# facebookresearch/ReAgent

Measured on NVIDIA H100. Metric: minibatch_td_updates_per_sec_b4096, higher is better.
Workload: dtype f32

## Files before the change

### include/reagent_b200.h

```cpp
#ifndef REAGENT_B200_H_
#define REAGENT_B200_H_

#include <stdint.h>

#ifdef __cplusplus
extern "C" {
#endif

#define RB200_VERSION 1
#define RB200_MAX_LAYERS 8

#define RB200_OK 0
#define RB200_E_INVALID (-1)
#define RB200_E_CUDA (-2)
#define RB200_E_SMEM (-3)

#define RB200_ACT_LINEAR 0
#define RB200_ACT_RELU 1
#define RB200_ACT_TANH 2
#define RB200_ACT_LEAKY_RELU 3
#define RB200_ACT_SIGMOID 4
#define RB200_ACT_SOFTPLUS 5

#define RB200_LOSS_MSE 0
// ... 270 lines not shown
#define RB200_ALGO_TD3 1
typedef struct rb200_ac_args {
  int32_t batch;
  int32_t algo;
  const float* state;
  const float* action;
  const float* next_state;
  const float* reward;
  const float* not_terminal;
  const float* noise_next;
  const float* noise_cur;
  float gamma;
  const float* alpha;
  const float* log_alpha;
  float target_entropy;
  int32_t backprop_through_log_prob;
  float noise_variance, noise_clip;
  float* loss_partials;
  float* loss;
  uint32_t* tile_counter;
  float* alpha_grad;
  float* td_target;
  float* next_action_out;
  float* log_prob_out;
  float* q1_value;
  float* q2_value;
  const rb200_mlp_t* value_target;
  const rb200_mlp_t* value_net;
  float* min_q_out;
  int32_t crr_mode;
  float crr_threshold;
  float crr_beta;
  float crr_clamp;
  int32_t logged_action_uniform_prior;
  const float* sample_weight;
  float* td_error_out;
} rb200_ac_args_t;
#define RB200_CRR_NONE 0
#define RB200_CRR_INDICATOR 1
#define RB200_CRR_EXPONENT 2

int rb200_ac_critic_step(const rb200_mlp_t* actor, const rb200_mlp_t* q1, const rb200_mlp_t* q2,
                         const rb200_mlp_t* q1_target, const rb200_mlp_t* q2_target,
                         const rb200_ac_args_t* args, const rb200_net_ws_t* ws_q1,
                         const rb200_net_ws_t* ws_q2, void* stream);
int rb200_ac_actor_step(const rb200_mlp_t* actor, const rb200_mlp_t* q1, const rb200_mlp_t* q2,
                        const rb200_ac_args_t* args, const rb200_net_ws_t* ws_actor,
                        const rb200_net_ws_t* ws_q1, const rb200_net_ws_t* ws_q2, void* stream);
int rb200_ac_value_step(const rb200_mlp_t* value, const rb200_ac_args_t* args,
                        const rb200_net_ws_t* ws_value, void* stream);

int rb200_wgrad_splits(int batch);
int rb200_wgrad_splits_for(const rb200_mlp_t* net, int32_t batch);
int rb200_mlp_wgrad(const rb200_mlp_t* net, const float* net_input, int32_t batch,
                    const rb200_net_ws_t* ws, float* gpart, int32_t splits, void* stream);
int rb200_grad_reduce(const float* gpart, int32_t splits, int64_t n, float* g, void* stream);

typedef struct rb200_adam_args {
  float* params;
  const float* grad;
  int32_t splits;
  int64_t n;
  float* exp_avg;
  float* exp_avg_sq;
  int64_t* step;
  uint32_t* block_counter;
  double lr, beta1, beta2, eps, weight_decay;
  float grad_scale;
  float* target;
  float tau;
  float one_minus_tau;
  float* exp_out;
  const rb200_mlp_t* tc_net;
  void* tc_pack_ws;
  int64_t tc_pack_ws_bytes;
  int32_t tc_do_backward;
  int32_t dp_world, dp_rank;
  float* const* dp_recv;
  uint32_t* const* dp_flags;
  int64_t dp_stride;
  int32_t dp_max_blocks;
  int32_t decoupled_weight_decay;
  int32_t amsgrad;
  float* max_exp_avg_sq;
} rb200_adam_args_t;
int rb200_adam_blocks(int64_t n);
int rb200_adam_soft_update(const rb200_adam_args_t* a, void* stream);
int rb200_soft_update(float* target, const float* source, int64_t n, float tau,
                      float one_minus_tau, void* stream);


#define RB200_SAMPLE_PRIORITIZED 0
#define RB200_SAMPLE_UNIFORM 1
#define RB200_SAMPLE_GIVEN 2
#define RB200_VALID_BLOCK 256
#define RB200_MAX_GATHER_SPECS 12

typedef struct rb200_gather_spec {
  const void* src;
  void* dst;
  int32_t row_bytes;
  int32_t which;
} rb200_gather_spec_t;

typedef struct rb200_sample_args {
  int32_t batch, capacity, update_horizon, mode;
// ... 127 lines not shown
```

### reagent_b200/_lib.py

```python
import ctypes as C
import os

MAX_LAYERS = 8

ACT = {"linear": 0, "relu": 1, "tanh": 2, "leaky_relu": 3, "sigmoid": 4, "softplus": 5}
E_SMEM = -3
LOSS_MSE, LOSS_HUBER = 0, 1
DISCOUNT_CONST, DISCOUNT_POW = 0, 1

_f32p = C.POINTER(C.c_float)
_vp = C.c_void_p


class MlpT(C.Structure):
    _fields_ = [
        ("n_layers", C.c_int32),
        ("dims", C.c_int32 * (MAX_LAYERS + 1)),
        ("act", C.c_int32 * MAX_LAYERS),
        ("params", _vp),
        ("w_off", C.c_int64 * MAX_LAYERS),
        ("b_off", C.c_int64 * MAX_LAYERS),
        ("n_params", C.c_int64),
    ]

# ... 240 lines not shown
    lib.rb200_device_info.argtypes = [C.POINTER(C.c_int), C.POINTER(C.c_int)]
    lib.rb200_num_row_tiles.argtypes = [C.c_int, C.c_int, C.c_int]
    lib.rb200_dqn_td_step.argtypes = [C.POINTER(MlpT), C.POINTER(MlpT), C.POINTER(DqnArgsT),
                                      C.POINTER(NetWsT), _vp]
    lib.rb200_dueling_scratch_floats.argtypes = [C.c_int32, C.c_int32]
    lib.rb200_dueling_scratch_floats.restype = C.c_int64
    lib.rb200_dueling_fold.argtypes = [_vp, _vp, _vp, _vp, C.c_int32, C.c_int32, C.c_int32, _vp, _vp,
                                       _vp, _vp]
    lib.rb200_dueling_unfold.argtypes = [_vp, C.c_int64, C.c_int32, C.c_int32, C.c_int32, C.c_int32,
                                         C.c_int64, C.c_int64, C.c_int64, C.c_int64, C.c_int64,
                                         C.c_int64, _vp, _vp]
    lib.rb200_dqn_tc_workspace_bytes.argtypes = [C.POINTER(MlpT), C.c_int32, C.c_int32]
    lib.rb200_dqn_tc_workspace_bytes.restype = C.c_int64
    lib.rb200_dqn_tc_pack.argtypes = [C.POINTER(MlpT), C.POINTER(MlpT), C.c_int32, C.c_int32, _vp,
                                      C.c_int64, _vp]
    lib.rb200_dqn_td_step_tc.argtypes = [C.POINTER(MlpT), C.POINTER(MlpT), C.POINTER(DqnArgsT),
                                         C.POINTER(NetWsT), _vp, C.c_int64, C.c_int32, _vp]
    lib.rb200_mlp_forward.argtypes = [C.POINTER(MlpT), _vp, C.c_int32, _vp, C.c_int32, C.c_int32,
                                      _vp, C.POINTER(NetWsT), _vp]
    lib.rb200_mlp_forward_tiled.argtypes = [C.POINTER(MlpT), C.POINTER(MlpT), _vp, C.c_int32, _vp,
                                            C.c_int32, C.c_int32, C.c_int32, _vp, _vp, _vp]
    lib.rb200_linear_forward.argtypes = [_vp, _vp, C.c_int32, C.c_int32, C.c_int32, _vp,
                                         C.c_int32, _vp, _vp]
    lib.rb200_linear_backward_dx.argtypes = [_vp, C.c_int32, C.c_int32, _vp, _vp, C.c_int32,
                                             C.c_int32, _vp, _vp]
    lib.rb200_linear_backward_dx_tc_scratch_bytes.argtypes = [C.c_int32, C.c_int32, C.c_int32]
    lib.rb200_linear_backward_dx_tc_scratch_bytes.restype = C.c_int64
    lib.rb200_linear_backward_dx_tc.argtypes = [_vp, C.c_int32, C.c_int32, _vp, _vp, C.c_int32,
                                                C.c_int32, _vp, _vp, C.c_int64, _vp]
    lib.rb200_mlp_backward.argtypes = [C.POINTER(MlpT), _vp, C.c_int32, C.POINTER(NetWsT), _vp]
    lib.rb200_qrdqn_head.argtypes = [C.POINTER(QrdqnArgsT), _vp]
    lib.rb200_preprocess.argtypes = [_vp, _vp, C.c_int32, C.c_int64, C.c_int32, C.c_int32, _vp,
                                     _vp, _vp, _vp]
    lib.rb200_replay_sample.argtypes = [C.POINTER(SampleArgsT), _vp]
    lib.rb200_valid_index_build.argtypes = [_vp, C.c_int64, _vp, _vp, _vp]
    lib.rb200_mt19937_uniform_host.argtypes = [_vp, C.POINTER(C.c_int32), _vp, _vp, _vp, C.c_int64]
    lib.rb200_mt19937_uniform_host.restype = None
    lib.rb200_sumtree_set_host.argtypes = [_vp, C.c_int32, _vp, _vp, C.c_int64, _vp]
    lib.rb200_sumtree_sample_host.argtypes = [_vp, C.c_int32, C.c_double]
    lib.rb200_sumtree_sample_host.restype = C.c_int64
    lib.rb200_sumtree_sample_many_host.argtypes = [_vp, C.c_int32, _vp, _vp, C.c_int64, _vp]
    lib.rb200_sumtree_sample_many_host.restype = None
    lib.rb200_replay_add_batch_host.argtypes = [_vp, C.c_int64, C.c_int64, C.c_int32, _vp, _vp, _vp]
    lib.rb200_replay_add_batch_host.restype = None
    lib.rb200_ac_critic_step.argtypes = [C.POINTER(MlpT), C.POINTER(MlpT), C.POINTER(MlpT),
                                         C.POINTER(MlpT), C.POINTER(MlpT), C.POINTER(AcArgsT),
                                         C.POINTER(NetWsT), C.POINTER(NetWsT), _vp]
    lib.rb200_ac_actor_step.argtypes = [C.POINTER(MlpT), C.POINTER(MlpT), C.POINTER(MlpT),
                                        C.POINTER(AcArgsT), C.POINTER(NetWsT), C.POINTER(NetWsT),
                                        C.POINTER(NetWsT), _vp]
    lib.rb200_ac_value_step.argtypes = [C.POINTER(MlpT), C.POINTER(AcArgsT), C.POINTER(NetWsT), _vp]
    lib.rb200_wgrad_splits.argtypes = [C.c_int]
    lib.rb200_wgrad_splits_for.argtypes = [C.POINTER(MlpT), C.c_int32]
    lib.rb200_mlp_wgrad.argtypes = [C.POINTER(MlpT), _vp, C.c_int32, C.POINTER(NetWsT), _vp,
                                    C.c_int32, _vp]
    lib.rb200_grad_reduce.argtypes = [_vp, C.c_int32, C.c_int64, _vp, _vp]
    lib.rb200_adam_soft_update.argtypes = [C.POINTER(AdamArgsT), _vp]
    lib.rb200_soft_update.argtypes = [_vp, _vp, C.c_int64, C.c_float, C.c_float, _vp]
    lib.rb200_cpe_heads.argtypes = [C.POINTER(CpeArgsT), _vp]
    lib.rb200_bcq_filter.argtypes = [_vp, C.c_int32, C.c_int32, C.c_float, _vp, _vp, _vp, _vp, _vp]
    lib.rb200_pdqn_head.argtypes = [C.POINTER(PdqnArgsT), _vp]
    lib.rb200_c51_head.argtypes = [C.POINTER(C51ArgsT), _vp]
    lib.rb200_bc_xent_head.argtypes = [C.POINTER(BcXentArgsT), _vp]
    lib.rb200_crr_critic_head.argtypes = [C.POINTER(CrrCriticArgsT), _vp]
    lib.rb200_crr_actor_head.argtypes = [C.POINTER(CrrActorArgsT), _vp]
    lib.rb200_replay_add_device.argtypes = [C.POINTER(AddArgsT), _vp]
    lib.rb200_sumtree_set_device.argtypes = [_vp, C.c_int32, _vp, _vp, C.c_int32, _vp, _vp, _vp]
    lib.rb200_per_draw_indices.argtypes = [C.POINTER(PerDrawArgsT), _vp]
    lib.rb200_per_weights.argtypes = [_vp, C.c_int32, _vp, C.c_int32, _vp, C.c_double, C.c_double,
                                      _vp, _vp, _vp]
    lib.rb200_per_priority_update.argtypes = [_vp, C.c_int32, _vp, _vp, _vp, C.c_int32, C.c_double,
                                              C.c_double, _vp, _vp, _vp, _vp]
    lib.rb200_per_priority_update_rows.argtypes = [_vp, C.c_int32, _vp, _vp, C.c_int32, C.c_double,
                                                   C.c_double, C.c_double, _vp, _vp, _vp, _vp]
    lib.rb200_adam_blocks.argtypes = [C.c_int64]
    lib.rb200_dp_alloc.argtypes = [C.c_int64, C.POINTER(_vp)]
    lib.rb200_dp_free.argtypes = [_vp]
    lib.rb200_dp_ipc_handle.argtypes = [_vp, _vp]
    lib.rb200_dp_ipc_open.argtypes = [_vp, C.POINTER(_vp)]
    lib.rb200_dp_ipc_close.argtypes = [_vp]


def lib():
    global _LIB
    if _LIB is None:
        if not os.path.exists(LIB_PATH):
            raise Rb200Error(
                f"{LIB_PATH} not found: the CUDA extension is not built. "
                "Run reagent_b200/csrc/build.sh (there is no CPU fallback).")
        _LIB = C.CDLL(LIB_PATH)
        _declare(_LIB)
    return _LIB


def check(rc, what=""):
    if rc != 0:
        msg = lib().rb200_last_error().decode("utf-8", "replace")
        raise Rb200Error(f"{what} failed (rc={rc}): {msg}")


def ptr(t, device=None):
    if t is None:
        return None
    if not t.is_cuda:
        raise Rb200Error("reagent_b200: a CPU tensor reached a CUDA entry point (call "
                         "trainer.cuda() / batch.cuda() first; there is no CPU path)")
# ... 25 lines not shown
```

### reagent_b200/csrc/rb200_optim.cu

```cuda
#include <math.h>

#include <stdlib.h>

#include "rb200_dqn_tc_layout.cuh"

namespace rb200 {

constexpr int kWgTile = 64;
constexpr int kWgRows = 32;
constexpr int kWgLd = kWgTile + 8;

struct WgradLayer {
  const float* A;
  const float* dZ;
  int K, N;
  long long w_off, b_off;
  int tiles_n, tiles_k, tile_start;
};
struct WgradParams {
  int n_layers;
  WgradLayer L[kMaxLayers];
  int B, splits, rows_per_split;
  float* gpart;
  long long P;
// ... 273 lines not shown
    m = w1_small ? fmaf(w1, gm, m) : fmaf(w1m1, gm, g);
    v = __fadd_rn(__fmul_rn(v, b2), __fmul_rn(__fmul_rn(w2, g), g));
    float vd = v;
    if (kAmsgrad) {
      vd = fmax_nan(a.max_exp_avg_sq[i], v);
      a.max_exp_avg_sq[i] = vd;
    }
    const float denom = __fadd_rn(__fdiv_rn(__fsqrt_rn(vd), bc2_sqrt), eps);
    p = __fadd_rn(p, __fdiv_rn(__fmul_rn(-step_size, m), denom));
    a.params[i] = p;
    a.exp_avg[i] = m;
    a.exp_avg_sq[i] = v;
    if (a.exp_out) a.exp_out[i] = expf(p);
    float tn = 0.f;
    if (a.target) {
      const float tg = a.target[i];
      tn = __fadd_rn(__fmul_rn(a.tau, p), __fmul_rn(a.one_minus_tau, tg));
      a.target[i] = tn;
    }
    if (d.pv.pack) adam_pack_weight(d.pv, i, p, a.target != nullptr, tn);
  }
  __syncthreads();
  if (threadIdx.x == 0) {
    __threadfence();
    const unsigned done = atomicAdd(a.block_counter, 1u);
    if (done == gridDim.x - 1) {
      *a.step = t;
      *a.block_counter = 0u;
    }
  }
}

__global__ void soft_update_kernel(float* __restrict__ target, const float* __restrict__ src,
                                   long long n, float tau, float omt) {
  const long long stride = (long long)gridDim.x * blockDim.x;
  for (long long i = (long long)blockIdx.x * blockDim.x + threadIdx.x; i < n; i += stride)
    target[i] = __fadd_rn(__fmul_rn(tau, src[i]), __fmul_rn(omt, target[i]));
}

}

using namespace rb200;

extern "C" int rb200_wgrad_splits(int batch) {
  const char* e = getenv("RB200_WGRAD_ROWS");
  int rows = e ? atoi(e) : 256;
  if (rows < 32) rows = 32;
  int s = batch / rows;
  if (s < 1) s = 1;
  if (s > 64) s = 64;
  return s;
}

int rb200_wgrad_tc_launch(const rb200_mlp_t* net, const float* net_input, int32_t batch,
                          const rb200_net_ws_t* ws, float* gpart, int32_t splits, void* stream);

static bool wgrad_use_tc() {
  const char* d = getenv("RB200_DISABLE_WGMMA");
  const char* w = getenv("RB200_WGRAD_TC");
  return !(d && d[0] && d[0] != '0') && (w && w[0] == '1');
}

extern "C" int rb200_wgrad_splits_for(const rb200_mlp_t* net, int32_t batch) {
  if (!net || !wgrad_use_tc()) return rb200_wgrad_splits(batch);
  int jobs = 0;
  for (int l = 0; l < net->n_layers; ++l) jobs += ceil_div(net->dims[l + 1], 128) * ceil_div(net->dims[l], 256);
  int s = ceil_div(2 * kNumSMs, jobs < 1 ? 1 : jobs);
  const int smax = batch / 128 < 1 ? 1 : batch / 128;
  if (s > smax) s = smax;
  if (s > 64) s = 64;
  return s < 1 ? 1 : s;
}

extern "C" int rb200_mlp_wgrad(const rb200_mlp_t* net, const float* net_input, int32_t batch,
                               const rb200_net_ws_t* ws, float* gpart, int32_t splits,
                               void* stream) {
  if (!net || !ws || !gpart) { set_last_error("rb200_mlp_wgrad: null argument"); return RB200_E_INVALID; }
  if (int rc = validate_mlp(net, "net")) return rc;
  if (batch <= 0 || splits <= 0) { set_last_error("rb200_mlp_wgrad: bad batch/splits"); return RB200_E_INVALID; }
  if (wgrad_use_tc()) return rb200_wgrad_tc_launch(net, net_input, batch, ws, gpart, splits, stream);
  WgradParams p = {};
  p.n_layers = net->n_layers;
  p.B = batch;
  p.splits = splits;
  p.rows_per_split = ceil_div(ceil_div(batch, splits), kWgRows) * kWgRows;
  p.gpart = gpart;
  p.P = net->n_params;
  int tiles = 0;
  for (int l = 0; l < net->n_layers; ++l) {
    WgradLayer& L = p.L[l];
    L.A = (l == 0) ? (net_input ? net_input : ws->input) : ws->hidden[l - 1];
    L.dZ = ws->dz[l];
    if (!L.A || !L.dZ) { set_last_error("rb200_mlp_wgrad: missing activation / dz for layer %d", l); return RB200_E_INVALID; }
    L.K = net->dims[l];
    L.N = net->dims[l + 1];
    L.w_off = net->w_off[l];
    L.b_off = net->b_off[l];
    L.tiles_n = ceil_div(L.N, kWgTile);
    L.tiles_k = ceil_div(L.K, kWgTile);
    L.tile_start = tiles;
    tiles += L.tiles_n * L.tiles_k;
  }
  for (int l = net->n_layers; l < kMaxLayers; ++l) p.L[l].tile_start = 1 << 30;
  dim3 grid(tiles, splits);
  wgrad_kernel<<<grid, kThreads, 0, (cudaStream_t)stream>>>(p);
  return check_cuda(cudaGetLastError(), "wgrad_kernel launch");
}

extern "C" int rb200_grad_reduce(const float* gpart, int32_t splits, int64_t n, float* g,
                                 void* stream) {
  if (!gpart || !g || n <= 0 || splits <= 0) { set_last_error("rb200_grad_reduce: bad argument"); return RB200_E_INVALID; }
  int blocks = (int)((n + 255) / 256);
  if (blocks > kNumSMs * 8) blocks = kNumSMs * 8;
  grad_reduce_kernel<<<blocks, 256, 0, (cudaStream_t)stream>>>(gpart, splits, (long long)n, g);
  return check_cuda(cudaGetLastError(), "grad_reduce_kernel launch");
}

extern "C" int rb200_adam_soft_update(const rb200_adam_args_t* a, void* stream) {
  if (!a || !a->params || !a->grad || !a->exp_avg || !a->exp_avg_sq || !a->step || !a->block_counter) {
    set_last_error("rb200_adam_soft_update: null argument"); return RB200_E_INVALID;
  }
  if (a->n <= 0 || a->splits <= 0) { set_last_error("rb200_adam_soft_update: bad n/splits"); return RB200_E_INVALID; }
  if ((a->decoupled_weight_decay != 0 && a->decoupled_weight_decay != 1) ||
      (a->amsgrad != 0 && a->amsgrad != 1)) {
    set_last_error("rb200_adam_soft_update: decoupled_weight_decay and amsgrad must be 0 or 1"); return RB200_E_INVALID;
  }
  if (a->amsgrad && !a->max_exp_avg_sq) { set_last_error("rb200_adam_soft_update: amsgrad needs max_exp_avg_sq"); return RB200_E_INVALID; }
  AdamDev d;
  d.a = *a;
  d.a.tc_net = nullptr;
  d.pv.pack = nullptr;
  if (a->tc_net && a->tc_pack_ws) {
    const rb200_mlp_t* q = a->tc_net;
// ... 47 lines not shown
```

### reagent_b200/csrc/rb200_wgrad_tc.cu

```cuda
#include "rb200_wgmma.cuh"

namespace rb200 {

constexpr int kWtRows = 32;
constexpr int kWtM = 128;
constexpr int kWtN = 256;
constexpr int kWtQuadA = kWtM * 16 + 16;
constexpr int kWtQuadB = kWtN * 16 + 16;
constexpr int kWtPlaneA = (kWtRows / 4) * kWtQuadA;
constexpr int kWtPlaneB = (kWtRows / 4) * kWtQuadB;
constexpr int kWtStage = 2 * (kWtPlaneA + kWtPlaneB);
constexpr int kWtThreads = 256;
constexpr int kWtSmem = 2 * kWtStage + 64;

struct WtLayer {
  const float* A;
  const float* dZ;
  int K, N;
  long long w_off, b_off;
  int tiles_m, tiles_k, job_start;
};
struct WtParams {
  int n_layers;
  WtLayer L[kMaxLayers];
  int B, rows_per_split;
  float* gpart;
  long long P;
};

template <int NT>
__device__ __forceinline__ void wt_kstep(float* acc, uint64_t dah, uint64_t dal, uint64_t dbh,
                                         uint64_t dbl) {
  if constexpr (NT == 32) {
    wgmma_ss_n32(acc, dah, dbh, 1u); wgmma_ss_n32(acc, dal, dbh, 1u); wgmma_ss_n32(acc, dah, dbl, 1u);
  } else if constexpr (NT == 64) {
    wgmma_ss_n64(acc, dah, dbh, 1u); wgmma_ss_n64(acc, dal, dbh, 1u); wgmma_ss_n64(acc, dah, dbl, 1u);
  } else if constexpr (NT == 128) {
    wgmma_ss_n128(acc, dah, dbh, 1u); wgmma_ss_n128(acc, dal, dbh, 1u); wgmma_ss_n128(acc, dah, dbl, 1u);
  } else {
    wgmma_ss_n256(acc, dah, dbh, 1u); wgmma_ss_n256(acc, dal, dbh, 1u); wgmma_ss_n256(acc, dah, dbl, 1u);
  }
}

__global__ void __launch_bounds__(kWtThreads, 1) wgrad_tc_kernel(const WtParams p) {
  extern __shared__ __align__(128) unsigned char smem[];
  const int tid = threadIdx.x, warp = tid >> 5, lane = tid & 31;
  const int wg = warp >> 2;
  int li = 0;
  while (li + 1 < p.n_layers && (int)blockIdx.x >= p.L[li + 1].job_start) ++li;
  const WtLayer& Ly = p.L[li];
  const int job = blockIdx.x - Ly.job_start;
  const int tm = job / Ly.tiles_k, tk = job - tm * Ly.tiles_k;
  const int n0 = tm * kWtM, k0 = tk * kWtN;
  const int N = Ly.N, K = Ly.K;
  const int nrows_m = min(kWtM, N - n0);
  const int ncols = min(kWtN, K - k0);
  const int n_mma = ncols <= 32 ? 32 : (ncols <= 64 ? 64 : (ncols <= 128 ? 128 : 256));
  const int split = blockIdx.y;
  const int b_begin = split * p.rows_per_split;
  const int b_end = min(p.B, b_begin + p.rows_per_split);
  const int nchunks = ceil_div(max(b_end - b_begin, 0), kWtRows);


  const int fa = (nrows_m + 7) & ~7, fb = (ncols + 7) & ~7;
  const int ua = 2 * (fa / 8), utotal = ua + 2 * (fb / 8);
  constexpr int kMaxUnits = (2 * (kWtM / 8) + 2 * (kWtN / 8)) / (kWtThreads / 32);
  const int r_l = lane & 15, qsel = lane >> 4;
  float4 regs[kMaxUnits];
  auto chunk_fetch = [&](int c) {
    const int r0 = b_begin + c * kWtRows;
#pragma unroll
    for (int u = 0; u < kMaxUnits; ++u) {
      const int unit = warp + u * (kWtThreads / 32);
      float4 v = make_float4(0.f, 0.f, 0.f, 0.f);
      if (unit < utotal) {
        const bool isb = unit >= ua;
        const int j = isb ? unit - ua : unit;
        const int h = j & 1, fp = j >> 1;
        const int row = r0 + 16 * h + r_l;
        const int f = (isb ? k0 : n0) + 8 * fp + 4 * qsel;
        const int F = isb ? K : N;
        if (row < b_end && f < F) {
          const float* src = (isb ? Ly.A : Ly.dZ) + (size_t)row * F + f;
          if (f + 3 < F && ((reinterpret_cast<uintptr_t>(src) & 15) == 0)) {
            v = __ldg(reinterpret_cast<const float4*>(src));
          } else {
            v.x = src[0];
            if (f + 1 < F) v.y = src[1];
            if (f + 2 < F) v.z = src[2];
            if (f + 3 < F) v.w = src[3];
          }
        }
      }
      regs[u] = v;
    }
  };
  auto chunk_store = [&](int st) {
    unsigned char* base = smem + st * kWtStage;
#pragma unroll
    for (int u = 0; u < kMaxUnits; ++u) {
      const int unit = warp + u * (kWtThreads / 32);
      if (unit >= utotal) continue;
      const bool isb = unit >= ua;
      const int j = isb ? unit - ua : unit;
      const int h = j & 1, fp = j >> 1;
      const int r = 16 * h + r_l;
      const int fl = 8 * fp + 4 * qsel;
      float* hi = reinterpret_cast<float*>(base + (isb ? 2 * kWtPlaneA + (r >> 2) * kWtQuadB
                                                       : (r >> 2) * kWtQuadA) + fl * 16) + (r & 3);
      float* lo = reinterpret_cast<float*>(reinterpret_cast<unsigned char*>(hi) + (isb ? kWtPlaneB : kWtPlaneA));
      float4 hh, ll;
      split4(regs[u], hh, ll);
      hi[0] = hh.x; hi[4] = hh.y; hi[8] = hh.z; hi[12] = hh.w;
      lo[0] = ll.x; lo[4] = ll.y; lo[8] = ll.z; lo[12] = ll.w;
    }
  };
  float bsum = 0.f;
  auto chunk_bias = [&](int st) {
    if (tk != 0 || tid >= kWtM) return;
    const unsigned char* base = smem + st * kWtStage;
#pragma unroll
    for (int rq = 0; rq < kWtRows / 4; ++rq) {
      const float4 a = *reinterpret_cast<const float4*>(base + rq * kWtQuadA + tid * 16);
      const float4 b = *reinterpret_cast<const float4*>(base + kWtPlaneA + rq * kWtQuadA + tid * 16);
      bsum += ((a.x + b.x) + (a.y + b.y)) + ((a.z + b.z) + (a.w + b.w));
    }
  };

  float acc[kWtN / 2];
#pragma unroll
  for (int i = 0; i < kWtN / 2; ++i) acc[i] = 0.f;
  auto chunk_mma = [&](int st) {
    const uint32_t sb = smem_u32(smem + st * kWtStage);
    const uint32_t a_hi = sb + (uint32_t)wg * 64 * 16, a_lo = a_hi + kWtPlaneA;
    const uint32_t b_hi = sb + 2 * kWtPlaneA, b_lo = b_hi + kWtPlaneB;
    wgmma_fence();
#pragma unroll
    for (int ks = 0; ks < kWtRows / 8; ++ks) {
      const uint32_t oa = ks * 2 * kWtQuadA, ob = ks * 2 * kWtQuadB;
      const uint64_t dah = wgmma_desc(a_hi + oa, kWtQuadA, 128), dal = wgmma_desc(a_lo + oa, kWtQuadA, 128);
      const uint64_t dbh = wgmma_desc(b_hi + ob, kWtQuadB, 128), dbl = wgmma_desc(b_lo + ob, kWtQuadB, 128);
      switch (n_mma) {
        case 32: wt_kstep<32>(acc, dah, dal, dbh, dbl); break;
        case 64: wt_kstep<64>(acc, dah, dal, dbh, dbl); break;
        case 128: wt_kstep<128>(acc, dah, dal, dbh, dbl); break;
        default: wt_kstep<256>(acc, dah, dal, dbh, dbl); break;
      }
    }
    wgmma_commit();
  };

  if (nchunks > 0) chunk_fetch(0);
  for (int c = 0; c < nchunks; ++c) {
    const int st = c & 1;
    chunk_store(st);
    if (c + 1 < nchunks) chunk_fetch(c + 1);
    fence_proxy_async_smem();
    __syncthreads();
    chunk_bias(st);
    chunk_mma(st);
    wgmma_wait<1>();
    __syncthreads();
  }
  wgmma_wait<0>();
  __syncthreads();

  float* gp = p.gpart + (size_t)split * p.P;
  constexpr int kLdT = kWtN + 4;
  float* tile = reinterpret_cast<float*>(smem);
  {
    const int r = wg * 64 + (warp & 3) * 16 + (lane >> 2);
    const int cq = 2 * (lane & 3);
#pragma unroll
    for (int j = 0; j < kWtN / 8; ++j) {
      if (8 * j < n_mma) {
        *reinterpret_cast<float2*>(tile + (size_t)r * kLdT + 8 * j + cq) = make_float2(acc[4 * j], acc[4 * j + 1]);
        *reinterpret_cast<float2*>(tile + (size_t)(r + 8) * kLdT + 8 * j + cq) =
            make_float2(acc[4 * j + 2], acc[4 * j + 3]);
      }
    }
  }
  if (tid < kWtM && tk == 0 && n0 + tid < N) gp[Ly.b_off + n0 + tid] = bsum;
  __syncthreads();
  {
    const bool v4 = ((K & 3) == 0) && ((k0 & 3) == 0) && ((Ly.w_off & 3) == 0) &&
                    ((reinterpret_cast<uintptr_t>(gp) & 15) == 0);
    for (int r = warp; r < nrows_m; r += kWtThreads / 32) {
      float* dst = gp + Ly.w_off + (size_t)(n0 + r) * K + k0;
      const float* src = tile + (size_t)r * kLdT;
      if (v4) {
        for (int c = lane * 4; c < ncols; c += 128)
          *reinterpret_cast<float4*>(dst + c) = *reinterpret_cast<const float4*>(src + c);
      } else {
        for (int c = lane; c < ncols; c += 32) dst[c] = src[c];
      }
    }
  }
}

}

using namespace rb200;

int rb200_wgrad_tc_launch(const rb200_mlp_t* net, const float* net_input, int32_t batch,
                          const rb200_net_ws_t* ws, float* gpart, int32_t splits, void* stream) {
  WtParams p = {};
  p.n_layers = net->n_layers;
  p.B = batch;
  p.rows_per_split = ceil_div(ceil_div(batch, splits), kWtRows) * kWtRows;
  p.gpart = gpart;
  p.P = net->n_params;
  int jobs = 0;
  for (int l = 0; l < net->n_layers; ++l) {
    WtLayer& L = p.L[l];
    L.A = (l == 0) ? (net_input ? net_input : ws->input) : ws->hidden[l - 1];
    L.dZ = ws->dz[l];
    if (!L.A || !L.dZ) { set_last_error("rb200_mlp_wgrad: missing activation / dz for layer %d", l); return RB200_E_INVALID; }
    L.K = net->dims[l];
    L.N = net->dims[l + 1];
    L.w_off = net->w_off[l];
    L.b_off = net->b_off[l];
    L.tiles_m = ceil_div(L.N, kWtM);
    L.tiles_k = ceil_div(L.K, kWtN);
    L.job_start = jobs;
    jobs += L.tiles_m * L.tiles_k;
  }
  for (int l = net->n_layers; l < kMaxLayers; ++l) p.L[l].job_start = 1 << 30;
  dim3 grid(jobs, splits);
  return launch<wgrad_tc_kernel>(grid, kWtThreads, kWtSmem, (cudaStream_t)stream,
                                 "wgrad_tc_kernel launch", p);
}
```

Baseline: 9945.

## Replace opt-in wgrad TC kernel with producer-fed wgmma kernel enabled by default

Removes the old opt-in 256-thread wgmma wgrad kernel and adds a warp-specialized kernel. One producer warp streams batch chunks through a 3-stage cp.async/mbarrier ring while four consumer warps split fp32 into hi/lo and run register-sourced wgmma on 64x64 tiles. The new path is used by default when the shapes fit and the job count stays within the SM count, and split selection goes back to the generic row-based heuristic. This aims to overlap global loads with tensor-core work and raise occupancy, at the cost of extra hi/lo split arithmetic and smem traffic per chunk, plus a shape gate that may fall back to the mma.sync path.

```diff
diff --git a/include/reagent_b200.h b/include/reagent_b200.h
--- a/include/reagent_b200.h
+++ b/include/reagent_b200.h
@@ -346,6 +346,7 @@
 
 int rb200_wgrad_splits(int batch);
 int rb200_wgrad_splits_for(const rb200_mlp_t* net, int32_t batch);
+int rb200_wgrad_uses_wgmma(const rb200_mlp_t* net, const float* net_input, const rb200_net_ws_t* ws);
 int rb200_mlp_wgrad(const rb200_mlp_t* net, const float* net_input, int32_t batch,
                     const rb200_net_ws_t* ws, float* gpart, int32_t splits, void* stream);
 int rb200_grad_reduce(const float* gpart, int32_t splits, int64_t n, float* g, void* stream);
diff --git a/profiles/time_wgrad.py b/profiles/time_wgrad.py
--- /dev/null
+++ b/profiles/time_wgrad.py
@@ -0,0 +1,158 @@
+import argparse
+import os
+import sys
+
+ROOT = os.path.dirname(os.path.dirname(os.path.abspath(__file__)))
+if ROOT not in sys.path:
+    sys.path.insert(0, ROOT)
+
+from profiles.timing import alternate, capture, card_info, cuda_device, replay_us, write_result
+
+NETS = {
+    "config2_q": ([128, 256, 128, 16], 4096),
+    "config3_qrdqn": ([128, 256, 128, 32 * 200], 4096),
+    "config4_sac_critic": ([256 + 32, 256, 256, 1], 8192),
+    "config4_sac_actor": ([256, 256, 256, 64], 8192),
+    "config5_td3_critic": ([512 + 64, 256, 256, 1], 16384),
+    "config5_td3_actor": ([512, 256, 256, 64], 16384),
+}
+SWEEP = (4, 8, 11, 16, 22, 32)
+
+
+class Problem:
+
+    def __init__(self, dims, batch, dev, seed=0):
+        import torch
+
+        from reagent_b200 import _lib
+        from reagent_b200.models.arena import ParamArena
+
+        self.dims, self.batch = dims, batch
+        L = len(dims) - 1
+        acts = [_lib.ACT["relu"]] * (L - 1) + [_lib.ACT["linear"]]
+        ar = ParamArena(dims, acts)
+        self.w_off, self.b_off, self.n, self.acts = list(ar.w_off), list(ar.b_off), ar.n, acts
+        g = torch.Generator(device=dev).manual_seed(seed)
+        self.params = torch.randn(self.n, device=dev, generator=g) * 0.05
+        self.target = self.params.clone()
+        self.exp_avg, self.exp_avg_sq = torch.zeros_like(self.params), torch.zeros_like(self.params)
+        self.step = torch.zeros(1, dtype=torch.int64, device=dev)
+        self.counter = torch.zeros(1, dtype=torch.int32, device=dev)
+        self.a = [torch.randn(batch, dims[l], device=dev, generator=g) for l in range(L)]
+        self.dz = [torch.randn(batch, dims[l + 1], device=dev, generator=g) for l in range(L)]
+        self.ws = _lib.NetWsT()
+        for l in range(1, L):
+            self.ws.hidden[l - 1] = self.a[l].data_ptr()
+        for l in range(L):
+            self.ws.dz[l] = self.dz[l].data_ptr()
+        self.gparts = {}
+
+    def desc(self):
+        from reagent_b200 import _lib
+
+        d = _lib.MlpT()
+        d.n_layers = len(self.dims) - 1
+        for i, v in enumerate(self.dims):
+            d.dims[i] = v
+        for i, (w, b, act) in enumerate(zip(self.w_off, self.b_off, self.acts)):
+            d.act[i], d.w_off[i], d.b_off[i] = act, w, b
+        d.params = self.params.data_ptr()
+        d.n_params = self.n
+        return d
+
+    def gpart(self, splits):
+        import torch
+
+        if splits not in self.gparts:
+            self.gparts[splits] = torch.zeros(splits, self.n, device=self.params.device)
+        return self.gparts[splits]
+
+    def wgrad(self, splits):
+        from reagent_b200 import _lib
+
+        _lib.check(_lib.lib().rb200_mlp_wgrad(self.desc(), self.a[0].data_ptr(), self.batch,
+                                              self.ws, self.gpart(splits).data_ptr(), splits,
+                                              _lib.cur_stream()), "rb200_mlp_wgrad")
+
+    def adam(self, splits):
+        from reagent_b200 import _lib
+
+        a = _lib.AdamArgsT()
+        a.params, a.grad, a.splits, a.n = self.params.data_ptr(), self.gpart(splits).data_ptr(), splits, self.n
+        a.exp_avg, a.exp_avg_sq = self.exp_avg.data_ptr(), self.exp_avg_sq.data_ptr()
+        a.step, a.block_counter = self.step.data_ptr(), self.counter.data_ptr()
+        a.lr, a.beta1, a.beta2, a.eps = 1e-3, 0.9, 0.999, 1e-8
+        a.weight_decay, a.grad_scale = 0.0, 1.0 / self.batch
+        a.decoupled_weight_decay, a.amsgrad, a.max_exp_avg_sq = 0, 0, None
+        a.target, a.tau, a.one_minus_tau = self.target.data_ptr(), 0.005, 0.995
+        a.exp_out, a.dp_world = None, 1
+        _lib.check(_lib.lib().rb200_adam_soft_update(a, _lib.cur_stream()), "rb200_adam_soft_update")
+
+
+def graph(fn, launches, mma_sync):
+    if mma_sync:
+        os.environ["RB200_DISABLE_WGMMA"] = "1"
+    try:
+        return capture(fn, launches)
+    finally:
+        os.environ.pop("RB200_DISABLE_WGMMA", None)
+
+
+def main():
+    ap = argparse.ArgumentParser()
+    ap.add_argument("--out", required=True, help="directory for the result file")
+    ap.add_argument("--reps", type=int, default=11)
+    ap.add_argument("--launches", type=int, default=200)
+    args = ap.parse_args()
+
+    dev = cuda_device(__file__)
+    from reagent_b200 import _lib
+
+    lib = _lib.lib()
+    info = card_info()
+    os.environ.pop("RB200_DISABLE_WGMMA", None)
+
+    probs, graphs, splits = {}, {}, {}
+    for name, (dims, B) in NETS.items():
+        p = probs[name] = Problem(dims, B, dev)
+        s_old = s_new = lib.rb200_wgrad_splits_for(p.desc(), B)
+        splits[name] = {"mma_sync": s_old, "default": s_new}
+        graphs[(name, "mma_sync")] = graph(lambda p=p, s=s_old: p.wgrad(s), args.launches, True)
+        graphs[(name, "default")] = graph(lambda p=p, s=s_new: p.wgrad(s), args.launches, False)
+    alone = alternate(graphs, args.reps, lambda k, rep: replay_us(graphs[k], args.launches))
+    wgrad_alone = {name: {path: dict(splits=splits[name][path],
+                                     **{s: alone[(name, path)][s] for s in ("median", "min", "max")})
+                          for path in ("mma_sync", "default")} for name in NETS}
+    for name in NETS:
+        w = wgrad_alone[name]
+        w["mma_sync_over_default"] = w["mma_sync"]["median"] / w["default"]["median"]
+    del graphs
+
+    p = probs["config2_q"]
+    pair = lambda s: (lambda: (p.wgrad(s), p.adam(s)))
+    s_old = lib.rb200_wgrad_splits(p.batch)
+    variants = {f"wgmma_s{s}": graph(pair(s), args.launches, False) for s in SWEEP}
+    variants[f"mma_sync_s{s_old}"] = graph(pair(s_old), args.launches, True)
+    both = alternate(variants, args.reps, lambda k, rep: replay_us(variants[k], args.launches))
+
+    res = {
+        "what": ("rb200_mlp_wgrad alone on the networks of bench.py configs 2-5, mma.sync kernel "
+                 "against the default path (the producer-fed wgmma kernel where the shapes "
+                 "allow); wgrad + Adam (K3, with Polyak) on the config-2 q-network over slab "
+                 "counts"),
+        "card": info,
+        "nets": {k: dict(dims=v[0], batch=v[1]) for k, v in NETS.items()},
+        "method": (f"CUDA events around one replay of a graph of {args.launches} launches "
+                   f"(wgrad + Adam pairs in b), captured after 5 warm-up launches on a side "
+                   f"stream, after one untimed replay; {args.reps} alternating repetitions, "
+                   f"medians in microseconds per launch"),
+        "wgrad_alone_us": wgrad_alone,
+        "wgrad_plus_adam_config2_us": {k: {s: v[s] for s in ("median", "min", "max")}
+                                       for k, v in both.items()},
+        "splits_config2": splits["config2_q"]["default"],
+    }
+    write_result(args.out, __file__, res)
+
+
+if __name__ == "__main__":
+    main()
diff --git a/reagent_b200/_lib.py b/reagent_b200/_lib.py
--- a/reagent_b200/_lib.py
+++ b/reagent_b200/_lib.py
@@ -316,6 +316,7 @@
     lib.rb200_ac_value_step.argtypes = [C.POINTER(MlpT), C.POINTER(AcArgsT), C.POINTER(NetWsT), _vp]
     lib.rb200_wgrad_splits.argtypes = [C.c_int]
     lib.rb200_wgrad_splits_for.argtypes = [C.POINTER(MlpT), C.c_int32]
+    lib.rb200_wgrad_uses_wgmma.argtypes = [C.POINTER(MlpT), _vp, C.POINTER(NetWsT)]
     lib.rb200_mlp_wgrad.argtypes = [C.POINTER(MlpT), _vp, C.c_int32, C.POINTER(NetWsT), _vp,
                                     C.c_int32, _vp]
     lib.rb200_grad_reduce.argtypes = [_vp, C.c_int32, C.c_int64, _vp, _vp]
diff --git a/reagent_b200/csrc/rb200_optim.cu b/reagent_b200/csrc/rb200_optim.cu
--- a/reagent_b200/csrc/rb200_optim.cu
+++ b/reagent_b200/csrc/rb200_optim.cu
@@ -349,24 +349,25 @@
   return s;
 }
 
-int rb200_wgrad_tc_launch(const rb200_mlp_t* net, const float* net_input, int32_t batch,
-                          const rb200_net_ws_t* ws, float* gpart, int32_t splits, void* stream);
-
-static bool wgrad_use_tc() {
+bool rb200_wgrad_wgmma_fits(const rb200_mlp_t* net, const float* net_input, const rb200_net_ws_t* ws);
+int rb200_wgrad_jobs(const rb200_mlp_t* net);
+int rb200_wgrad_wgmma_launch(const rb200_mlp_t* net, const float* net_input, int32_t batch,
+                             const rb200_net_ws_t* ws, float* gpart, int32_t splits, void* stream);
+
+static bool wgrad_use_wgmma(const rb200_mlp_t* net, const float* net_input, const rb200_net_ws_t* ws) {
   const char* d = getenv("RB200_DISABLE_WGMMA");
-  const char* w = getenv("RB200_WGRAD_TC");
-  return !(d && d[0] && d[0] != '0') && (w && w[0] == '1');
+  if (d && d[0] && d[0] != '0') return false;
+  return rb200_wgrad_wgmma_fits(net, net_input, ws) && rb200_wgrad_jobs(net) <= kNumSMs;
+}
+
+extern "C" int rb200_wgrad_uses_wgmma(const rb200_mlp_t* net, const float* net_input,
+                                      const rb200_net_ws_t* ws) {
+  return net && ws && validate_mlp(net, "net") == 0 && wgrad_use_wgmma(net, net_input, ws) ? 1 : 0;
 }
 
 extern "C" int rb200_wgrad_splits_for(const rb200_mlp_t* net, int32_t batch) {
-  if (!net || !wgrad_use_tc()) return rb200_wgrad_splits(batch);
-  int jobs = 0;
-  for (int l = 0; l < net->n_layers; ++l) jobs += ceil_div(net->dims[l + 1], 128) * ceil_div(net->dims[l], 256);
-  int s = ceil_div(2 * kNumSMs, jobs < 1 ? 1 : jobs);
-  const int smax = batch / 128 < 1 ? 1 : batch / 128;
-  if (s > smax) s = smax;
-  if (s > 64) s = 64;
-  return s < 1 ? 1 : s;
+  (void)net;
+  return rb200_wgrad_splits(batch);
 }
 
 extern "C" int rb200_mlp_wgrad(const rb200_mlp_t* net, const float* net_input, int32_t batch,
@@ -375,7 +376,8 @@
   if (!net || !ws || !gpart) { set_last_error("rb200_mlp_wgrad: null argument"); return RB200_E_INVALID; }
   if (int rc = validate_mlp(net, "net")) return rc;
   if (batch <= 0 || splits <= 0) { set_last_error("rb200_mlp_wgrad: bad batch/splits"); return RB200_E_INVALID; }
-  if (wgrad_use_tc()) return rb200_wgrad_tc_launch(net, net_input, batch, ws, gpart, splits, stream);
+  if (wgrad_use_wgmma(net, net_input, ws))
+    return rb200_wgrad_wgmma_launch(net, net_input, batch, ws, gpart, splits, stream);
   WgradParams p = {};
   p.n_layers = net->n_layers;
   p.B = batch;
diff --git a/reagent_b200/csrc/rb200_wgrad.cu b/reagent_b200/csrc/rb200_wgrad.cu
--- /dev/null
+++ b/reagent_b200/csrc/rb200_wgrad.cu
@@ -0,0 +1,271 @@
+#include "rb200_wgmma.cuh"
+
+namespace rb200 {
+
+constexpr int kWrRows = 32;
+constexpr int kWrTile = 64;
+constexpr int kWrSub = 32;
+constexpr int kWrLd = kWrTile + 8;
+constexpr int kWrStages = 3;
+constexpr int kWrFactor = kWrRows * kWrLd * 4;
+constexpr int kWrStage = 2 * kWrFactor;
+constexpr int kWrQuad = 2 * kWrTile * 16;
+constexpr int kWrPlane = (kWrRows / 4) * kWrQuad;
+constexpr int kWrConsumers = 128;
+constexpr int kWrThreads = kWrConsumers + 32;
+constexpr int kWrBars = kWrStages * kWrStage + kWrPlane;
+constexpr int kWrSmem = kWrBars + 2 * kWrStages * 8;
+constexpr int kWrLdT = kWrTile + 4;
+static_assert(kWrTile * kWrLdT * 4 <= kWrStages * kWrStage, "epilogue tile fits in the ring");
+
+struct WrLayer {
+  const float* X;
+  const float* Y;
+  int FX, FY;
+  int swap;
+  int K;
+  long long w_off, b_off;
+  int tiles_y, job_start;
+};
+struct WrParams {
+  int n_layers;
+  WrLayer L[kMaxLayers];
+  int B, rows_per_split;
+  float* gpart;
+  long long P;
+};
+
+__device__ __forceinline__ void wr_split(float x, uint32_t& hi, uint32_t& lo) {
+  hi = (__float_as_uint(x) + 0x1000u) & 0xffffe000u;
+  lo = __float_as_uint(x - __uint_as_float(hi));
+}
+__device__ __forceinline__ void wr_consumer_sync() {
+  asm volatile("bar.sync 1, %0;\n" ::"n"(kWrConsumers) : "memory");
+}
+
+__global__ void __launch_bounds__(kWrThreads, 3) wgrad_wgmma_kernel(const WrParams p) {
+  extern __shared__ __align__(128) unsigned char smem[];
+  uint64_t* full = reinterpret_cast<uint64_t*>(smem + kWrBars);
+  uint64_t* sfree = full + kWrStages;
+  const int tid = threadIdx.x;
+  int li = 0;
+  while (li + 1 < p.n_layers && (int)blockIdx.x >= p.L[li + 1].job_start) ++li;
+  const WrLayer& Ly = p.L[li];
+  const int job = blockIdx.x - Ly.job_start;
+  const int tx = job / Ly.tiles_y, ty = job - tx * Ly.tiles_y;
+  const int x0 = tx * kWrTile, y0 = ty * kWrTile;
+  const int wx = min(kWrTile, Ly.FX - x0), wy = min(kWrTile, Ly.FY - y0);
+  const int split = blockIdx.y;
+  const int b_begin = split * p.rows_per_split;
+  const int b_end = min(p.B, b_begin + p.rows_per_split);
+  const int nchunks = ceil_div(max(b_end - b_begin, 0), kWrRows);
+
+  if (tid == 0) {
+    for (int s = 0; s < kWrStages; ++s) { mbar_init(full + s, 32); mbar_init(sfree + s, kWrConsumers); }
+    asm volatile("fence.mbarrier_init.release.cluster;\n" ::: "memory");
+  }
+  __syncthreads();
+
+  if (tid >= kWrConsumers) {
+    const int lane = tid - kWrConsumers;
+    for (int c = 0; c < nchunks; ++c) {
+      const int s = c % kWrStages;
+      if (c >= kWrStages) mbar_wait(sfree + s, (c / kWrStages - 1) & 1);
+      const int r0 = b_begin + c * kWrRows;
+      const int nv = min(kWrRows, b_end - r0);
+      float* xs = reinterpret_cast<float*>(smem + s * kWrStage);
+      float* ys = reinterpret_cast<float*>(smem + s * kWrStage + kWrFactor);
+      for (int i = lane; i < nv * (kWrTile / 4); i += 32) {
+        const int r = i / (kWrTile / 4), f = 4 * (i % (kWrTile / 4));
+        if (f < wx) cp_async16(xs + r * kWrLd + f, Ly.X + (size_t)(r0 + r) * Ly.FX + x0 + f);
+        if (f < wy) cp_async16(ys + r * kWrLd + f, Ly.Y + (size_t)(r0 + r) * Ly.FY + y0 + f);
+      }
+      asm volatile("cp.async.mbarrier.arrive.noinc.shared::cta.b64 [%0];\n" ::"r"(smem_u32(full + s))
+                   : "memory");
+    }
+    asm volatile("cp.async.wait_all;\n" ::: "memory");
+    return;
+  }
+
+  const int warp = tid >> 5, lane = tid & 31, g = lane >> 2, q = lane & 3;
+  const int nsub = wy > kWrSub ? 2 : 1;
+  unsigned char* plane = smem + kWrStages * kWrStage;
+  const bool bias = Ly.swap ? tx == 0 : ty == 0;
+  const int bias_w = Ly.swap ? wy : wx;
+  float bsum = 0.f;
+  float acc[32];
+#pragma unroll
+  for (int i = 0; i < 32; ++i) acc[i] = 0.f;
+
+  for (int c = 0; c < nchunks; ++c) {
+    const int s = c % kWrStages;
+    const int nv = min(kWrRows, b_end - (b_begin + c * kWrRows));
+    mbar_wait(full + s, (c / kWrStages) & 1);
+    const float* xs = reinterpret_cast<const float*>(smem + s * kWrStage);
+    const float* ys = reinterpret_cast<const float*>(smem + s * kWrStage + kWrFactor);
+    uint32_t ah[4][4], al[4][4];
+#pragma unroll
+    for (int ks = 0; ks < 4; ++ks) {
+#pragma unroll
+      for (int i = 0; i < 4; ++i) {
+        const int r = 8 * ks + q + 4 * (i >> 1);
+        const float v = r < nv ? xs[r * kWrLd + 16 * warp + g + 8 * (i & 1)] : 0.f;
+        wr_split(v, ah[ks][i], al[ks][i]);
+      }
+    }
+#pragma unroll
+    for (int sb = 0; sb < 2; ++sb) {
+      if (sb < nsub) {
+        const int f = lane, fy = kWrSub * sb + f;
+#pragma unroll
+        for (int i = 0; i < 2; ++i) {
+          const int rq = warp + 4 * i;
+          float4 v = make_float4(0.f, 0.f, 0.f, 0.f);
+          if (fy < wy) {
+            const float* src = ys + 4 * rq * kWrLd + fy;
+            if (4 * rq + 0 < nv) v.x = src[0];
+            if (4 * rq + 1 < nv) v.y = src[kWrLd];
+            if (4 * rq + 2 < nv) v.z = src[2 * kWrLd];
+            if (4 * rq + 3 < nv) v.w = src[3 * kWrLd];
+          }
+          float4 hi, lo;
+          split4(v, hi, lo);
+          unsigned char* dst = plane + rq * kWrQuad;
+          *reinterpret_cast<float4*>(dst + fy * 16) = hi;
+          *reinterpret_cast<float4*>(dst + (kWrTile + fy) * 16) = lo;
+        }
+      }
+    }
+    if (bias && tid < bias_w) {
+      const float* zs = Ly.swap ? ys : xs;
+      for (int r = 0; r < nv; ++r) bsum += zs[r * kWrLd + tid];
+    }
+    mbar_arrive(sfree + s);
+    fence_proxy_async_smem();
+    wr_consumer_sync();
+    wgmma_fence();
+#pragma unroll
+    for (int ks = 0; ks < 4; ++ks) {
+      const uint32_t b = smem_u32(plane) + ks * 2 * kWrQuad;
+      const uint64_t bh = wgmma_desc(b, kWrQuad, 128), bl = wgmma_desc(b + kWrTile * 16, kWrQuad, 128);
+      if (nsub == 2) {
+        if (Ly.swap) {
+          wgmma_rs_n64(acc, ah[ks], bl, 1u);
+          wgmma_rs_n64(acc, al[ks], bh, 1u);
+        } else {
+          wgmma_rs_n64(acc, al[ks], bh, 1u);
+          wgmma_rs_n64(acc, ah[ks], bl, 1u);
+        }
+        wgmma_rs_n64(acc, ah[ks], bh, 1u);
+      } else {
+        if (Ly.swap) {
+          wgmma_rs_n32(acc, ah[ks], bl, 1u);
+          wgmma_rs_n32(acc, al[ks], bh, 1u);
+        } else {
+          wgmma_rs_n32(acc, al[ks], bh, 1u);
+          wgmma_rs_n32(acc, ah[ks], bl, 1u);
+        }
+        wgmma_rs_n32(acc, ah[ks], bh, 1u);
+      }
+    }
+    wgmma_commit();
+    wgmma_wait<0>();
+    wr_consumer_sync();
+  }
+
+  float* gp = p.gpart + (size_t)split * p.P;
+  float* tile = reinterpret_cast<float*>(smem);
+#pragma unroll
+  for (int j = 0; j < 8; ++j) {
+    if (j < 4 * nsub) {
+#pragma unroll
+      for (int h = 0; h < 2; ++h)
+#pragma unroll
+        for (int e = 0; e < 2; ++e) {
+          const int m = 16 * warp + g + 8 * h, n = 8 * j + 2 * q + e;
+          tile[Ly.swap ? n * kWrLdT + m : m * kWrLdT + n] = acc[4 * j + 2 * h + e];
+        }
+    }
+  }
+  if (bias && tid < bias_w) gp[Ly.b_off + (Ly.swap ? y0 : x0) + tid] = bsum;
+  wr_consumer_sync();
+  const int orow0 = Ly.swap ? y0 : x0, nrows = Ly.swap ? wy : wx;
+  const int ocol0 = Ly.swap ? x0 : y0, ncols = Ly.swap ? wx : wy;
+  const bool v4 = ((Ly.w_off & 3) == 0) && ((reinterpret_cast<uintptr_t>(gp) & 15) == 0);
+  for (int idx = tid; idx < nrows * (kWrTile / 4); idx += kWrConsumers) {
+    const int r = idx / (kWrTile / 4), c = 4 * (idx % (kWrTile / 4));
+    if (c >= ncols) continue;
+    const float4 v = *reinterpret_cast<const float4*>(tile + r * kWrLdT + c);
+    float* dst = gp + Ly.w_off + (size_t)(orow0 + r) * Ly.K + ocol0 + c;
+    if (v4) {
+      *reinterpret_cast<float4*>(dst) = v;
+    } else {
+      dst[0] = v.x; dst[1] = v.y; dst[2] = v.z; dst[3] = v.w;
+    }
+  }
+}
+
+bool wr_swap(int K, int N) {
+  const long long keep = (long long)ceil_div(N, kWrTile) * kWrTile * ceil_div(K, kWrSub) * kWrSub;
+  const long long swap = (long long)ceil_div(K, kWrTile) * kWrTile * ceil_div(N, kWrSub) * kWrSub;
+  return swap < keep;
+}
+
+}
+
+using namespace rb200;
+
+static bool aligned16(const void* p) { return (reinterpret_cast<uintptr_t>(p) & 15) == 0; }
+
+bool rb200_wgrad_wgmma_fits(const rb200_mlp_t* net, const float* net_input, const rb200_net_ws_t* ws) {
+  for (int l = 0; l < net->n_layers; ++l) {
+    if ((net->dims[l] & 3) || (net->dims[l + 1] & 3)) return false;
+    if (!ws) continue;
+    const float* A = (l == 0) ? (net_input ? net_input : ws->input) : ws->hidden[l - 1];
+    if (!aligned16(A) || !aligned16(ws->dz[l])) return false;
+  }
+  return true;
+}
+
+int rb200_wgrad_jobs(const rb200_mlp_t* net) {
+  int jobs = 0;
+  for (int l = 0; l < net->n_layers; ++l) {
+    const int K = net->dims[l], N = net->dims[l + 1];
+    const bool sw = wr_swap(K, N);
+    jobs += ceil_div(sw ? K : N, kWrTile) * ceil_div(sw ? N : K, kWrTile);
+  }
+  return jobs;
+}
+
+int rb200_wgrad_wgmma_launch(const rb200_mlp_t* net, const float* net_input, int32_t batch,
+                             const rb200_net_ws_t* ws, float* gpart, int32_t splits, void* stream) {
+  WrParams p = {};
+  p.n_layers = net->n_layers;
+  p.B = batch;
+  p.rows_per_split = ceil_div(ceil_div(batch, splits), kWrRows) * kWrRows;
+  p.gpart = gpart;
+  p.P = net->n_params;
+  int jobs = 0;
+  for (int l = 0; l < net->n_layers; ++l) {
+    const float* A = (l == 0) ? (net_input ? net_input : ws->input) : ws->hidden[l - 1];
+    const float* dZ = ws->dz[l];
+    if (!A || !dZ) { set_last_error("rb200_mlp_wgrad: missing activation / dz for layer %d", l); return RB200_E_INVALID; }
+    const int K = net->dims[l], N = net->dims[l + 1];
+    WrLayer& L = p.L[l];
+    L.swap = wr_swap(K, N) ? 1 : 0;
+    L.X = L.swap ? A : dZ;
+    L.Y = L.swap ? dZ : A;
+    L.FX = L.swap ? K : N;
+    L.FY = L.swap ? N : K;
+    L.K = K;
+    L.w_off = net->w_off[l];
+    L.b_off = net->b_off[l];
+    L.tiles_y = ceil_div(L.FY, kWrTile);
+    L.job_start = jobs;
+    jobs += ceil_div(L.FX, kWrTile) * L.tiles_y;
+  }
+  for (int l = net->n_layers; l < kMaxLayers; ++l) p.L[l].job_start = 1 << 30;
+  dim3 grid(jobs, splits);
+  return launch<wgrad_wgmma_kernel>(grid, kWrThreads, kWrSmem, (cudaStream_t)stream,
+                                    "wgrad_wgmma_kernel launch", p);
+}
diff --git a/reagent_b200/csrc/rb200_wgrad_tc.cu b/reagent_b200/csrc/rb200_wgrad_tc.cu
--- a/reagent_b200/csrc/rb200_wgrad_tc.cu
+++ /dev/null
@@ -1,232 +0,0 @@
-#include "rb200_wgmma.cuh"
-
-namespace rb200 {
-
-constexpr int kWtRows = 32;
-constexpr int kWtM = 128;
-constexpr int kWtN = 256;
-constexpr int kWtQuadA = kWtM * 16 + 16;
-constexpr int kWtQuadB = kWtN * 16 + 16;
-constexpr int kWtPlaneA = (kWtRows / 4) * kWtQuadA;
-constexpr int kWtPlaneB = (kWtRows / 4) * kWtQuadB;
-constexpr int kWtStage = 2 * (kWtPlaneA + kWtPlaneB);
-constexpr int kWtThreads = 256;
-constexpr int kWtSmem = 2 * kWtStage + 64;
-
-struct WtLayer {
-  const float* A;
-  const float* dZ;
-  int K, N;
-  long long w_off, b_off;
-  int tiles_m, tiles_k, job_start;
-};
-struct WtParams {
-  int n_layers;
-  WtLayer L[kMaxLayers];
-  int B, rows_per_split;
-  float* gpart;
-  long long P;
-};
-
-template <int NT>
-__device__ __forceinline__ void wt_kstep(float* acc, uint64_t dah, uint64_t dal, uint64_t dbh,
-                                         uint64_t dbl) {
-  if constexpr (NT == 32) {
-    wgmma_ss_n32(acc, dah, dbh, 1u); wgmma_ss_n32(acc, dal, dbh, 1u); wgmma_ss_n32(acc, dah, dbl, 1u);
-  } else if constexpr (NT == 64) {
-    wgmma_ss_n64(acc, dah, dbh, 1u); wgmma_ss_n64(acc, dal, dbh, 1u); wgmma_ss_n64(acc, dah, dbl, 1u);
-  } else if constexpr (NT == 128) {
-    wgmma_ss_n128(acc, dah, dbh, 1u); wgmma_ss_n128(acc, dal, dbh, 1u); wgmma_ss_n128(acc, dah, dbl, 1u);
-  } else {
-    wgmma_ss_n256(acc, dah, dbh, 1u); wgmma_ss_n256(acc, dal, dbh, 1u); wgmma_ss_n256(acc, dah, dbl, 1u);
-  }
-}
-
-__global__ void __launch_bounds__(kWtThreads, 1) wgrad_tc_kernel(const WtParams p) {
-  extern __shared__ __align__(128) unsigned char smem[];
-  const int tid = threadIdx.x, warp = tid >> 5, lane = tid & 31;
-  const int wg = warp >> 2;
-  int li = 0;
-  while (li + 1 < p.n_layers && (int)blockIdx.x >= p.L[li + 1].job_start) ++li;
-  const WtLayer& Ly = p.L[li];
-  const int job = blockIdx.x - Ly.job_start;
-  const int tm = job / Ly.tiles_k, tk = job - tm * Ly.tiles_k;
-  const int n0 = tm * kWtM, k0 = tk * kWtN;
-  const int N = Ly.N, K = Ly.K;
-  const int nrows_m = min(kWtM, N - n0);
-  const int ncols = min(kWtN, K - k0);
-  const int n_mma = ncols <= 32 ? 32 : (ncols <= 64 ? 64 : (ncols <= 128 ? 128 : 256));
-  const int split = blockIdx.y;
-  const int b_begin = split * p.rows_per_split;
-  const int b_end = min(p.B, b_begin + p.rows_per_split);
-  const int nchunks = ceil_div(max(b_end - b_begin, 0), kWtRows);
-
-
-  const int fa = (nrows_m + 7) & ~7, fb = (ncols + 7) & ~7;
-  const int ua = 2 * (fa / 8), utotal = ua + 2 * (fb / 8);
-  constexpr int kMaxUnits = (2 * (kWtM / 8) + 2 * (kWtN / 8)) / (kWtThreads / 32);
-  const int r_l = lane & 15, qsel = lane >> 4;
-  float4 regs[kMaxUnits];
-  auto chunk_fetch = [&](int c) {
-    const int r0 = b_begin + c * kWtRows;
-#pragma unroll
-    for (int u = 0; u < kMaxUnits; ++u) {
-      const int unit = warp + u * (kWtThreads / 32);
-      float4 v = make_float4(0.f, 0.f, 0.f, 0.f);
-      if (unit < utotal) {
-        const bool isb = unit >= ua;
-        const int j = isb ? unit - ua : unit;
-        const int h = j & 1, fp = j >> 1;
-        const int row = r0 + 16 * h + r_l;
-        const int f = (isb ? k0 : n0) + 8 * fp + 4 * qsel;
-        const int F = isb ? K : N;
-        if (row < b_end && f < F) {
-          const float* src = (isb ? Ly.A : Ly.dZ) + (size_t)row * F + f;
-          if (f + 3 < F && ((reinterpret_cast<uintptr_t>(src) & 15) == 0)) {
-            v = __ldg(reinterpret_cast<const float4*>(src));
-          } else {
-            v.x = src[0];
-            if (f + 1 < F) v.y = src[1];
-            if (f + 2 < F) v.z = src[2];
-            if (f + 3 < F) v.w = src[3];
-          }
-        }
-      }
-      regs[u] = v;
-    }
-  };
-  auto chunk_store = [&](int st) {
-    unsigned char* base = smem + st * kWtStage;
-#pragma unroll
-    for (int u = 0; u < kMaxUnits; ++u) {
-      const int unit = warp + u * (kWtThreads / 32);
-      if (unit >= utotal) continue;
-      const bool isb = unit >= ua;
-      const int j = isb ? unit - ua : unit;
-      const int h = j & 1, fp = j >> 1;
-      const int r = 16 * h + r_l;
-      const int fl = 8 * fp + 4 * qsel;
-      float* hi = reinterpret_cast<float*>(base + (isb ? 2 * kWtPlaneA + (r >> 2) * kWtQuadB
-                                                       : (r >> 2) * kWtQuadA) + fl * 16) + (r & 3);
-      float* lo = reinterpret_cast<float*>(reinterpret_cast<unsigned char*>(hi) + (isb ? kWtPlaneB : kWtPlaneA));
-      float4 hh, ll;
-      split4(regs[u], hh, ll);
-      hi[0] = hh.x; hi[4] = hh.y; hi[8] = hh.z; hi[12] = hh.w;
-      lo[0] = ll.x; lo[4] = ll.y; lo[8] = ll.z; lo[12] = ll.w;
-    }
-  };
-  float bsum = 0.f;
-  auto chunk_bias = [&](int st) {
-    if (tk != 0 || tid >= kWtM) return;
-    const unsigned char* base = smem + st * kWtStage;
-#pragma unroll
-    for (int rq = 0; rq < kWtRows / 4; ++rq) {
-      const float4 a = *reinterpret_cast<const float4*>(base + rq * kWtQuadA + tid * 16);
-      const float4 b = *reinterpret_cast<const float4*>(base + kWtPlaneA + rq * kWtQuadA + tid * 16);
-      bsum += ((a.x + b.x) + (a.y + b.y)) + ((a.z + b.z) + (a.w + b.w));
-    }
-  };
-
-  float acc[kWtN / 2];
-#pragma unroll
-  for (int i = 0; i < kWtN / 2; ++i) acc[i] = 0.f;
-  auto chunk_mma = [&](int st) {
-    const uint32_t sb = smem_u32(smem + st * kWtStage);
-    const uint32_t a_hi = sb + (uint32_t)wg * 64 * 16, a_lo = a_hi + kWtPlaneA;
-    const uint32_t b_hi = sb + 2 * kWtPlaneA, b_lo = b_hi + kWtPlaneB;
-    wgmma_fence();
-#pragma unroll
-    for (int ks = 0; ks < kWtRows / 8; ++ks) {
-      const uint32_t oa = ks * 2 * kWtQuadA, ob = ks * 2 * kWtQuadB;
-      const uint64_t dah = wgmma_desc(a_hi + oa, kWtQuadA, 128), dal = wgmma_desc(a_lo + oa, kWtQuadA, 128);
-      const uint64_t dbh = wgmma_desc(b_hi + ob, kWtQuadB, 128), dbl = wgmma_desc(b_lo + ob, kWtQuadB, 128);
-      switch (n_mma) {
-        case 32: wt_kstep<32>(acc, dah, dal, dbh, dbl); break;
-        case 64: wt_kstep<64>(acc, dah, dal, dbh, dbl); break;
-        case 128: wt_kstep<128>(acc, dah, dal, dbh, dbl); break;
-        default: wt_kstep<256>(acc, dah, dal, dbh, dbl); break;
-      }
-    }
-    wgmma_commit();
-  };
-
-  if (nchunks > 0) chunk_fetch(0);
-  for (int c = 0; c < nchunks; ++c) {
-    const int st = c & 1;
-    chunk_store(st);
-    if (c + 1 < nchunks) chunk_fetch(c + 1);
-    fence_proxy_async_smem();
-    __syncthreads();
-    chunk_bias(st);
-    chunk_mma(st);
-    wgmma_wait<1>();
-    __syncthreads();
-  }
-  wgmma_wait<0>();
-  __syncthreads();
-
-  float* gp = p.gpart + (size_t)split * p.P;
-  constexpr int kLdT = kWtN + 4;
-  float* tile = reinterpret_cast<float*>(smem);
-  {
-    const int r = wg * 64 + (warp & 3) * 16 + (lane >> 2);
-    const int cq = 2 * (lane & 3);
-#pragma unroll
-    for (int j = 0; j < kWtN / 8; ++j) {
-      if (8 * j < n_mma) {
-        *reinterpret_cast<float2*>(tile + (size_t)r * kLdT + 8 * j + cq) = make_float2(acc[4 * j], acc[4 * j + 1]);
-        *reinterpret_cast<float2*>(tile + (size_t)(r + 8) * kLdT + 8 * j + cq) =
-            make_float2(acc[4 * j + 2], acc[4 * j + 3]);
-      }
-    }
-  }
-  if (tid < kWtM && tk == 0 && n0 + tid < N) gp[Ly.b_off + n0 + tid] = bsum;
-  __syncthreads();
-  {
-    const bool v4 = ((K & 3) == 0) && ((k0 & 3) == 0) && ((Ly.w_off & 3) == 0) &&
-                    ((reinterpret_cast<uintptr_t>(gp) & 15) == 0);
-    for (int r = warp; r < nrows_m; r += kWtThreads / 32) {
-      float* dst = gp + Ly.w_off + (size_t)(n0 + r) * K + k0;
-      const float* src = tile + (size_t)r * kLdT;
-      if (v4) {
-        for (int c = lane * 4; c < ncols; c += 128)
-          *reinterpret_cast<float4*>(dst + c) = *reinterpret_cast<const float4*>(src + c);
-      } else {
-        for (int c = lane; c < ncols; c += 32) dst[c] = src[c];
-      }
-    }
-  }
-}
-
-}
-
-using namespace rb200;
-
-int rb200_wgrad_tc_launch(const rb200_mlp_t* net, const float* net_input, int32_t batch,
-                          const rb200_net_ws_t* ws, float* gpart, int32_t splits, void* stream) {
-  WtParams p = {};
-  p.n_layers = net->n_layers;
-  p.B = batch;
-  p.rows_per_split = ceil_div(ceil_div(batch, splits), kWtRows) * kWtRows;
-  p.gpart = gpart;
-  p.P = net->n_params;
-  int jobs = 0;
-  for (int l = 0; l < net->n_layers; ++l) {
-    WtLayer& L = p.L[l];
-    L.A = (l == 0) ? (net_input ? net_input : ws->input) : ws->hidden[l - 1];
-    L.dZ = ws->dz[l];
-    if (!L.A || !L.dZ) { set_last_error("rb200_mlp_wgrad: missing activation / dz for layer %d", l); return RB200_E_INVALID; }
-    L.K = net->dims[l];
-    L.N = net->dims[l + 1];
-    L.w_off = net->w_off[l];
-    L.b_off = net->b_off[l];
-    L.tiles_m = ceil_div(L.N, kWtM);
-    L.tiles_k = ceil_div(L.K, kWtN);
-    L.job_start = jobs;
-    jobs += L.tiles_m * L.tiles_k;
-  }
-  for (int l = net->n_layers; l < kMaxLayers; ++l) p.L[l].job_start = 1 << 30;
-  dim3 grid(jobs, splits);
-  return launch<wgrad_tc_kernel>(grid, kWtThreads, kWtSmem, (cudaStream_t)stream,
-                                 "wgrad_tc_kernel launch", p);
-}
```

Result: faster. 10190, median of 6 (+2.4%).
